# Lornatang/Real_ESRGAN-PyTorch

Measured on AMD Instinct MI355X. Metric: x4 SR train images/sec (256->1024), higher is better.
Workload: dtype f16; 1 GPU; RealESRNet x4 L1 train step, RRDBNet 23 blocks, LR 256^2 -> HR 1024^2, batch 16/GPU, degradation=hip, Adam+EMA, GradScaler; global_batch=16, parallelism=dp1

## Files before the change

include/resr.h:

```cpp
#ifndef RESR_H_
#define RESR_H_

#include <stddef.h>
#include <stdint.h>

#ifdef __cplusplus
extern "C" {
#endif

#define RESR_VERSION 3

typedef enum {
    RESR_OK = 0,
    RESR_ERR_ARG = -1,
    RESR_ERR_LAUNCH = -2,
    RESR_ERR_WORKSPACE = -3
} resr_status;

typedef enum { RESR_F16 = 0, RESR_F32 = 1, RESR_F16X2 = 2 } resr_dtype;

enum {
    RESR_CONV_LRELU = 1 << 0,
    RESR_CONV_UPSAMPLE_IN = 1 << 1,
    RESR_CONV_CLAMP01 = 1 << 2,
    RESR_CONV_OUT_NCHW_F32 = 1 << 3,
    RESR_CONV_MASK = 1 << 4,
    RESR_CONV_NO_BIAS = 1 << 5,
    RESR_CONV_AUX_BEFORE_MASK = 1 << 6,
    RESR_CONV_AUX_BEFORE_RES = 1 << 7,
    RESR_CONV_WRITE_SIGNBITS = 1 << 8,
    RESR_CONV_MASK_BITS = 1 << 9,
    RESR_CONV_OUT_SINGLE = 1 << 10,
    RESR_CONV_SINGLE_W16 = 1 << 11,
    RESR_CONV_MX_PAIRS = 1 << 12,
    RESR_CONV_MX_SIGNBITS = 1 << 13
};

typedef struct {
    int32_t n, h, w;
    int32_t cin;
    int32_t cin0;
    int32_t in0_stride;
    int32_t in1_stride;
    int32_t cout;
    int32_t cout_pad;
    int32_t out_stride;
    int32_t res0_stride, res1_stride, mask_stride;
    int32_t dtype;
    int32_t flags;
    float s0, t0, s1, t1, slope;
    int32_t in0_chunk_stride, in1_chunk_stride, out_chunk_stride;
    int32_t res0_chunk_stride, res1_chunk_stride, mask_chunk_stride;
    int64_t in0_lo_offset, in1_lo_offset, out_lo_offset, res0_lo_offset, res1_lo_offset;
    int32_t s2d_in_channels, s2d_out_channels, cout_groups;
    int32_t x2_pair_chunks;
    int32_t reserved2_;
    int64_t mask_lo_offset;
    int64_t in0_q_offset, in1_q_offset, out_q_offset, w_mx_offset;
// ... 370 lines not shown
```

real_esrgan-pytorch_amd/csrc/common.h:

```cpp
#pragma once
#include <hip/hip_runtime.h>
#include <stdint.h>
#include <stdio.h>
#include <stdlib.h>
#include <string.h>

#include <type_traits>

#include "resr.h"
#include "resr_debug.h"

namespace resr {

typedef _Float16 half_t;
typedef _Float16 half4 __attribute__((ext_vector_type(4)));
typedef _Float16 half8 __attribute__((ext_vector_type(8)));
typedef float float4v __attribute__((ext_vector_type(4)));
typedef unsigned uint2v __attribute__((ext_vector_type(2)));
typedef float float16v __attribute__((ext_vector_type(16)));

char* err_buf();
int fail(int code, const char* fmt, ...);

#define RESR_CHECK_LAUNCH(name)                                                        \
    do {                                                                               \
        hipError_t e_ = hipGetLastError();                                             \
        if (e_ != hipSuccess) return fail(RESR_ERR_LAUNCH, "%s: %s", name, hipGetErrorString(e_)); \
    } while (0)

bool prof_on();
void prof_before(hipStream_t st);
void prof_after(hipStream_t st, int kernel_id, double flop, double bytes = 0.0);

inline size_t elem_size(int dtype) { return dtype == RESR_F32 ? 4 : 2; }
inline size_t act_tensors(int dtype) { return dtype == RESR_F16X2 ? 2 : 1; }
constexpr float kLoScale = 4096.f, kLoInv = 1.f / 4096.f;
constexpr int kMaxDevices = 16;
inline size_t align_up(size_t v, size_t a) { return (v + a - 1) / a * a; }
inline bool no_pad_skip() { return getenv("RESR_NO_PAD_SKIP") != nullptr; }
inline bool degrade_parent_kernels() { return getenv("RESR_DEGRADE_PARENT_KERNELS") != nullptr; }

template <typename F>
inline bool with_scale(int s, F&& f) {
    switch (s) {
        case 1: f(std::integral_constant<int, 1>()); return true;
        case 2: f(std::integral_constant<int, 2>()); return true;
        case 3: f(std::integral_constant<int, 3>()); return true;
        case 4: f(std::integral_constant<int, 4>()); return true;
        default: return false;
    }
}

__device__ __forceinline__ void split_f16(float v, half_t& hi, half_t& lo) {
    hi = (half_t)v;
    lo = (half_t)((v - (float)hi) * kLoScale);
}

constexpr int kPrescaleBackoffStep = 4, kPrescaleBackoffMax = 40;
__host__ __device__ __forceinline__ bool grad_prescale_lifted(unsigned amax_bits) {
    const unsigned e = (amax_bits >> 23) & 0xffu;
    return e != 0u && e < 127u;
}
__host__ __device__ __forceinline__ float grad_prescale(unsigned amax_bits, bool inverse) {
// ... 58 lines not shown
```

real_esrgan-pytorch_amd/csrc/conv3x3.h:

```cpp
#pragma once
#include "host_api.h"

namespace resr {

struct ConvArgs {
    const char* in0;
    const char* in1;
    const char* w;
    const float* bias;
    const char* res0;
    const char* res1;
    const char* mask;
    char* out;
    uint8_t* aux;
    int n, h, w_, hs, ws;
    int cin, cin0;
    int in0_stride_b, in1_stride_b;
    int cout;
    int out_stride, res0_stride, res1_stride, mask_stride;
    size_t in0_chunk_b, in1_chunk_b;
    int out_chunk, res0_chunk, res1_chunk, mask_chunk;
    int flags;
    float s0, t0, s1, t1, slope;
    int tiles_x, tiles_y;
// ... 34 lines not shown
constexpr int kMaxChain = 6;
constexpr int kMaxBiasGroups = 8;
constexpr int kChainHdr = 16;
struct ChainArgs {
    int njobs;
    unsigned cap;
    unsigned* state;
    unsigned* host_errors;
    const char* nan16;
    int split[kMaxChain + 2];
    ChainJob job[kMaxChain];
};
struct ChainNone {};

bool conv3x3_ws_supported(const ConvArgs& a);
int conv3x3_ws_f16(const ConvArgs& a, int mt, bool x2, hipStream_t stream);
int conv3x3_ws_chain_f16(const ConvArgs& a, const ChainJob* jobs, int njobs, const double* flop, const double* bytes, bool x2, void* state, size_t state_bytes, hipStream_t stream);
int conv3x3_ws_mt1(const ConvArgs& a, int tile_rows, hipStream_t stream);
int conv3x3_ws_mt2(const ConvArgs& a, int tile_rows, hipStream_t stream);
int conv3x3_ws_x2_mt1(const ConvArgs& a, int tile_rows, hipStream_t stream);
int conv3x3_ws_x2_mt2(const ConvArgs& a, int tile_rows, hipStream_t stream);
int conv3x3_ws_mx_mt1(const ConvArgs& a, int tile_rows, hipStream_t stream);
int conv3x3_ws_mx_mt2(const ConvArgs& a, int tile_rows, hipStream_t stream);
int conv3x3_ws_sparse(const ConvArgs& a, int tile_rows, int sp, bool x2, hipStream_t stream);
int conv3x3_ws_chain_launch(const ConvArgs& a, const ChainArgs& cj, int tile_rows, int kind, bool x2, double flop, double bytes, hipStream_t stream);
int conv3x3_ws_chain_launch_x2(const ConvArgs& a, const ChainArgs& cj, int tile_rows, int kind, double flop, double bytes, hipStream_t stream);
int conv3x3_ws_chain_launch_mx(const ConvArgs& a, const ChainArgs& cj, int tile_rows, int kind, double flop, double bytes, hipStream_t stream);

inline ResrConvDesc conv_desc_base(int n, int h, int w, int dtype, int flags, float slope) {
    ResrConvDesc c;
    memset(&c, 0, sizeof(c));
    c.n = n; c.h = h; c.w = w; c.dtype = dtype; c.flags = flags;
    c.s0 = c.t0 = c.s1 = c.t1 = 1.f; c.slope = slope;
    return c;
}

inline double conv_algorithmic_bytes(const ConvArgs& a, size_t es) {
    const double px_out = (double)a.n * a.h * a.w_, px_in = (double)a.n * a.hs * a.ws;
    const int pair_ch = (es == 4 && a.pair_chunks > 0 && a.pair_chunks * 32 < a.cin) ? a.pair_chunks * 32 : a.cin;
    double b = px_in * (pair_ch * (double)es + (a.cin - pair_ch) * 2.0);
    const bool nchw = a.flags & RESR_CONV_OUT_NCHW_F32;
    b += px_out * a.cout * (nchw ? 4 : (es == 4 && a.out_single) ? 2 : es);
    if (a.flags & RESR_CONV_MASK) b += px_out * ((a.flags & RESR_CONV_MASK_BITS) ? ((a.cout + 31) / 32) * 4.0 : a.cout * (double)es);
    if (a.res0) b += px_out * a.cout * es;
    if (a.res1) b += px_out * a.cout * es;
    if (a.out_q) b += px_out * a.cout * 2.0;
    if (a.aux) b += px_out * ((a.flags & RESR_CONV_WRITE_SIGNBITS) ? ((a.cout + 31) / 32) * 4.0 : nchw ? a.cout : a.cout * (double)es);
    return b;
}

template <int SPP>
__device__ __forceinline__ int swz(int hx) {
    if constexpr (SPP == 4) return (hx >> 2) & 3;
    else return (hx >> 1) & 7;
}

template <typename T>
struct Frag;
template <>
struct Frag<half_t> {
    static __device__ __forceinline__ float16v mma(const uint4& a, const uint4& b, float16v c) {
        return __builtin_amdgcn_mfma_f32_32x32x16_f16(__builtin_bit_cast(half8, a),
                                                      __builtin_bit_cast(half8, b), c, 0, 0, 0);
    }
    static __device__ __forceinline__ float ld(const char* p, int idx) {
        return (float)reinterpret_cast<const half_t*>(p)[idx];
// ... 44 lines not shown
```

real_esrgan-pytorch_amd/csrc/conv3x3.hip:

```cpp
#include <stdlib.h>

#include <type_traits>

#include "conv3x3.h"
#include "packed_layout.h"

namespace resr {

template <typename T, int MT, int NT, int NW>
__global__ __launch_bounds__(64 * NW) void conv3x3_kernel(const ConvArgs a) {
    constexpr int NTHR = 64 * NW;
    constexpr int E = 16 / (int)sizeof(T);
    constexpr int SPP = 32 / E;
    constexpr int KS = SPP / 2;
    constexpr int PB = 32 * (int)sizeof(T);
    constexpr int TH = NW * NT, TW = 32, HH = TH + 2, HW = TW + 2;
    constexpr int NSLOT = HH * HW * SPP;
    constexpr int NS = (NSLOT + NTHR - 1) / NTHR;
    constexpr int BUF = HH * HW * PB;
    constexpr int WTAP = KS * MT * 1024;

    extern __shared__ __attribute__((aligned(16))) char smem[];

    const int tid = threadIdx.x, lane = tid & 63, wave = tid >> 6;
// ... 239 lines not shown
                        const float* bias, const void* res0, const void* res1, const void* mask,
                        void* out, void* aux, ConvArgs& a) {
    if (!d || !in0 || !w || !out) return fail(RESR_ERR_ARG, "conv3x3: null argument");
    if (d->cin <= 0 || (d->cin & 31) || (d->cin0 & 31) || d->cin0 <= 0 || d->cin0 > d->cin)
        return fail(RESR_ERR_ARG, "conv3x3: cin=%d cin0=%d must be positive multiples of 32", d->cin, d->cin0);
    if (d->cin0 < d->cin && !in1) return fail(RESR_ERR_ARG, "conv3x3: in1 missing for cin0 < cin");
    if (d->cout_pad != 32 && d->cout_pad != 64) return fail(RESR_ERR_ARG, "conv3x3: cout_pad=%d", d->cout_pad);
    if (d->cout <= 0 || d->cout > d->cout_pad) return fail(RESR_ERR_ARG, "conv3x3: cout=%d", d->cout);
    if (!(d->flags & RESR_CONV_OUT_NCHW_F32) && (d->cout & 3))
        return fail(RESR_ERR_ARG, "conv3x3: NHWC output needs cout %% 4 == 0");
    if (d->n <= 0 || d->h <= 0 || d->w <= 0) return fail(RESR_ERR_ARG, "conv3x3: empty shape");
    if ((d->flags & RESR_CONV_UPSAMPLE_IN) && ((d->h | d->w) & 1))
        return fail(RESR_ERR_ARG, "conv3x3: upsampled input needs even h,w");
    if ((d->flags & RESR_CONV_MASK) && !mask) return fail(RESR_ERR_ARG, "conv3x3: mask missing");
    if (d->flags & RESR_CONV_WRITE_SIGNBITS) {
        if (!aux || (d->cout & 7) || res0 || res1 ||
            (d->flags & (RESR_CONV_MASK | RESR_CONV_OUT_NCHW_F32 | RESR_CONV_CLAMP01 | RESR_CONV_AUX_BEFORE_MASK | RESR_CONV_AUX_BEFORE_RES)))
            return fail(RESR_ERR_ARG, "conv3x3: WRITE_SIGNBITS needs aux_out, cout %% 8 == 0 and a plain (bias/LeakyReLU) epilogue");
    }
    if (d->flags & RESR_CONV_MASK_BITS) {
        if (!(d->flags & RESR_CONV_MASK) || (d->cout & 7) || res0 || res1 || aux ||
            (d->flags & (RESR_CONV_OUT_NCHW_F32 | RESR_CONV_CLAMP01 | RESR_CONV_WRITE_SIGNBITS)))
            return fail(RESR_ERR_ARG, "conv3x3: MASK_BITS goes with MASK, cout %% 8 == 0, no residuals / aux");
    }
    const size_t es = elem_size(d->dtype);
    memset(&a, 0, sizeof(a));
    a.in0 = (const char*)in0; a.in1 = (const char*)in1; a.w = (const char*)w; a.bias = bias;
    a.res0 = (const char*)res0; a.res1 = (const char*)res1; a.mask = (const char*)mask;
    a.out = (char*)out; a.aux = (uint8_t*)aux;
    a.n = d->n; a.h = d->h; a.w_ = d->w;
    const bool up = d->flags & RESR_CONV_UPSAMPLE_IN;
    a.hs = up ? d->h / 2 : d->h; a.ws = up ? d->w / 2 : d->w;
    a.cin = d->cin; a.cin0 = d->cin0;
    a.in0_stride_b = (int)(d->in0_stride * es); a.in1_stride_b = (int)(d->in1_stride * es);
    a.cout = d->cout; a.out_stride = d->out_stride;
    a.res0_stride = d->res0_stride; a.res1_stride = d->res1_stride; a.mask_stride = d->mask_stride;
    auto chunk = [](int32_t v) { return v > 0 ? v : 32; };
    a.in0_chunk_b = (size_t)chunk(d->in0_chunk_stride) * es; a.in1_chunk_b = (size_t)chunk(d->in1_chunk_stride) * es;
    a.out_chunk = chunk(d->out_chunk_stride); a.res0_chunk = chunk(d->res0_chunk_stride);
    a.res1_chunk = chunk(d->res1_chunk_stride); a.mask_chunk = chunk(d->mask_chunk_stride);
    a.flags = d->flags & ~(RESR_CONV_OUT_SINGLE | RESR_CONV_SINGLE_W16 | RESR_CONV_MX_PAIRS | RESR_CONV_MX_SIGNBITS); a.s0 = d->s0; a.t0 = d->t0; a.s1 = d->s1; a.t1 = d->t1; a.slope = d->slope;
    a.s2d_c = 0; a.tap_c = 0; a.ngroups = 1; a.w_group_b = 0;
    a.pair_chunks = d->cin / 32; a.out_single = 0;
    a.mask_lo = (d->dtype == RESR_F16X2 && mask && (d->flags & RESR_CONV_MASK) && !(d->flags & RESR_CONV_MASK_BITS)) ? (long)d->mask_lo_offset : 0L;
    if (a.mask_lo < 0) return fail(RESR_ERR_ARG, "conv3x3: mask_lo_offset=%ld", a.mask_lo);
    if (d->dtype == RESR_F16X2) {
// ... 76 lines not shown
    const void* res0 = a.res0;
    const void* res1 = a.res1;
    const int groups = d->cout_groups > 1 ? d->cout_groups : 1;
    (void)have_bias;
    const int mt = d->cout_pad / 32;
    if (d->dtype == RESR_F16X2) {
        const bool nchw = d->flags & RESR_CONV_OUT_NCHW_F32;
        const bool in1_pairs = in1 && d->cin0 < d->cin && a.pair_chunks * 32 > d->cin0;
        if (d->in0_lo_offset == 0 || (in1_pairs && d->in1_lo_offset == 0) || (!nchw && !a.out_single && d->out_lo_offset == 0) ||
            (res0 && d->res0_lo_offset == 0) || (res1 && d->res1_lo_offset == 0))
            return fail(RESR_ERR_ARG, "conv3x3: RESR_F16X2 needs the hi -> lo offset of every pair operand");
        a.in0_lo_b = (size_t)d->in0_lo_offset * es; a.in1_lo_b = (size_t)d->in1_lo_offset * es;
        a.out_lo = a.out_single ? 0L : (long)d->out_lo_offset; a.res0_lo = (long)d->res0_lo_offset; a.res1_lo = (long)d->res1_lo_offset;
        if (!conv3x3_ws_supported(a))
            return fail(RESR_ERR_ARG, "conv3x3: RESR_F16X2 needs tensors below 4 GB / 2^24 pixels and cout %% 8 == 0");
        if (a.mx && (a.s2d_c > 0 || a.tap_c > 0)) return fail(RESR_ERR_ARG, "conv3x3: RESR_CONV_MX_PAIRS with sparse taps");
        return conv3x3_ws_f16(a, mt, true, stream);
    }
    const long tiles4 = (long)((d->w + 31) / 32) * ((d->h + 15) / 16) * d->n;
    const bool big = tiles4 >= 512;
    if (d->dtype == RESR_F16) {
        static const char* old_env = getenv("RESR_CONV_ONE_ROLE");
        if (!old_env && conv3x3_ws_supported(a)) return conv3x3_ws_f16(a, mt, false, stream);
        if (groups > 1) return fail(RESR_ERR_ARG, "conv3x3: cout_groups > 1 needs the producer/consumer kernel's preconditions");
        if (mt == 1) return big ? launch_conv<half_t, 1, 2, 8>(a, stream) : launch_conv<half_t, 1, 2, 4>(a, stream);
        return launch_conv<half_t, 2, 2, 4>(a, stream);
    } else if (d->dtype == RESR_F32) {
        if (mt == 1) return launch_conv<float, 1, 2>(a, stream);
        return launch_conv<float, 2, 2>(a, stream);
    }
    return fail(RESR_ERR_ARG, "conv3x3: dtype=%d", d->dtype);
}

int conv3x3_block_dispatch(int njobs, const ResrConvDesc* d, const void* in0, const void* in1, const void* const* w,
                           const float* const* bias, const void* const* mask, void* const* out, void* const* aux,
                           const ResrConvDesc* d5, const void* w5, const float* bias5, const void* res0_5, const void* res1_5,
                           void* out5, void* chain_state, size_t chain_state_bytes, hipStream_t stream) {
    if (njobs <= 0 || njobs > 4 || !d) return fail(RESR_ERR_ARG, "conv3x3_chain: njobs=%d", njobs);
    ConvArgs a[4], a5;
    for (int j = 0; j < njobs; ++j) {
        const int rc = conv3x3_args(&d[j], in0, in1, w[j], bias ? bias[j] : nullptr, nullptr, nullptr, mask ? mask[j] : nullptr,
                                    out[j], aux ? aux[j] : nullptr, a[j]);
        if (rc) return rc;
    }
    if (d5) {
        const int rc = conv3x3_args(d5, in0, in1, w5, bias5, res0_5, res1_5, nullptr, out5, nullptr, a5);
// ... 129 lines not shown
```

real_esrgan-pytorch_amd/csrc/conv3x3_ws.h:

```cpp
#pragma once
#include <stdlib.h>

#include <type_traits>

#include "conv3x3.h"

#ifndef RESR_TIMING_TAPS
#define RESR_TIMING_TAPS 9
#endif
#if defined(RESR_TRACE) && RESR_TRACE == 2
#define RESR_TRACE_STAMPS 192
#else
#define RESR_TRACE_STAMPS 64
#endif
#ifndef RESR_TIMING_VALU
#define RESR_TIMING_VALU 0
#endif

namespace resr {

static __device__ uint4 g_conv_zero16 = {0, 0, 0, 0};

extern unsigned long long* g_conv_trace;

// ... 176 lines not shown
    if (wave == 0 || wave == NWC) stamp(wave == 0 ? 1 : 0);

    float* bias_lds = reinterpret_cast<float*>(smem + C::NHB * BUF);
    if (wave == 0) {
        const bool f_bias = !(a.flags & RESR_CONV_NO_BIAS) && a.bias != nullptr;
        bias_lds[lane] = (f_bias && lane < a.cout) ? a.bias[lane] * (X2 ? kLoScale : 1.f) : 0.f;
    }
    if constexpr (MT == 2 && CH == 0) {
        if (a.ngroups > 1 && !(a.flags & RESR_CONV_NO_BIAS) && a.bias != nullptr) {
            float* gb = reinterpret_cast<float*>(smem + C::GB_OFF);
            for (int i = tid; i < a.ngroups * 64 && i < kMaxBiasGroups * 64; i += C::NTHR)
                gb[i] = a.bias[i] * (X2 ? kLoScale : 1.f);
        }
    }
    if constexpr (CH) {
        float* cb = reinterpret_cast<float*>(smem + C::CHAIN_OFF);
        if (wave < kMaxChain && lane < 32) {
            const float* bp = wave < cj.njobs ? cj.job[wave].bias : nullptr;
            cb[wave * 32 + lane] = (bp && !(a.flags & RESR_CONV_NO_BIAS) && lane < a.cout) ? bp[lane] * (X2 ? kLoScale : 1.f) : 0.f;
        }
        if (wave == 0 && lane == 0) *reinterpret_cast<unsigned*>(smem + C::CHAIN_OFF + kMaxChain * 128) = 0u;
    }
    constexpr bool FAST = EPI == 0 || EPI == 2 || EPI == 6 || EPI == 16 || EPI == 33 || EPI == 128;
    if constexpr (EPI == 128) {
        if (wave == 1) reinterpret_cast<float*>(smem + C::LUT_OFF)[lane] = lane < a.cout ? a.prelu[lane] : 0.f;
    }
    if constexpr (FAST && EPI == 33) {
        if (wave == 1 && lane < 16) {
            float4v m;
#pragma unroll
            for (int r = 0; r < 4; ++r) m[r] = (((lane >> r) & 1) ? 1.f : a.slope) * (X2 ? kLoInv : 1.f);
            *reinterpret_cast<float4v*>(smem + C::LUT_OFF + lane * 16) = m;
        }
    }
    if (wave >= NWC) {
        const int pw = wave - NWC;
        if constexpr (C::NHB == 3) {
            const int ups3 = (a.flags & RESR_CONV_UPSAMPLE_IN) ? 1 : 0;
            constexpr int REM = NI - (NIP - 1) * NP;
            static_assert(NIP < 64, "vmcnt is 6 bits");
            unsigned cst[NIP], pix[NIP];
            unsigned long long val[NIP], inb[NIP];
            const unsigned lds_base = (unsigned)(size_t)(__attribute__((address_space(3))) char*)smem;
            auto dma_s = [&](const char* sbase, unsigned voff, unsigned dst, unsigned long long mask) {
                unsigned long long save;
                asm volatile("s_mov_b64 %0, exec\n\ts_mov_b64 exec, %1\n\ts_mov_b32 m0, %2\n\ts_nop 0\n\t"
// ... 433 lines not shown
    int pend_tile = 0;
    unsigned pend_tag = 0;
    const int njobs_c = [&] { if constexpr (CH) return cj.njobs; else return 1; }();
    auto publish = [&]() {
        if constexpr (CH) {
            if (pend) {
                asm volatile("s_waitcnt vmcnt(0)" ::: "memory");
                if (lane == 0) {
                    unsigned* cnt = reinterpret_cast<unsigned*>(smem + C::CHAIN_OFF + kMaxChain * 128);
                    const unsigned old = __hip_atomic_fetch_add(cnt, 1u, __ATOMIC_RELAXED, __HIP_MEMORY_SCOPE_WORKGROUP);
                    if ((old % NWC) == NWC - 1)
                        __hip_atomic_store(cj.state + kChainHdr + pend_tile, pend_tag, __ATOMIC_RELAXED, __HIP_MEMORY_SCOPE_AGENT);
                }
                pend = false;
            }
        }
    };
    int c_tx = 0, c_ty = 0, c_n = 0, c_grp = 0;
    const int s_tx = tile_step % a.tiles_x, s_t2 = tile_step / a.tiles_x;
    const int s_ty = s_t2 % a.tiles_y, s_n = s_t2 / a.tiles_y;
    for (int job = (CH == 3 ? pin_job : 0); job < (CH == 3 ? pin_job + 1 : njobs_c); ++job) {
    if constexpr (CH) nchunks = stages_of(cj.job[job].cin);
    for (int tile = first; tile < tile_end; tile += tile_step) {
        if constexpr (FAST) {
            if (tile == first) {
                const int t2 = first / a.tiles_x;
                c_tx = first % a.tiles_x;
                c_ty = t2 % a.tiles_y;
                c_n = t2 / a.tiles_y;
            } else {
                c_tx += s_tx;
                if (c_tx >= a.tiles_x) { c_tx -= a.tiles_x; ++c_ty; }
                c_ty += s_ty;
                if (c_ty >= a.tiles_y) { c_ty -= a.tiles_y; ++c_n; }
                c_n += s_n;
            }
            c_grp = 0;
            if (MT == 2 && a.ngroups > 1) c_grp = c_n / a.n;
        }
        unsigned mword[EPI == 33 ? NT : 1][MT];
        bool own_top = true;
        if constexpr (CH == 2) own_top = cj.job[job].kind != 3;
        if constexpr (EPI == 33) if (own_top) {
            int x, y0, n;
            if constexpr (FAST) {
                x = c_tx * TW + (lane & 31);
                y0 = c_ty * TH + row0;
                n = c_n - c_grp * a.n;
            } else {
                const int tsp = tile % ntiles_sp;
                x = (tsp % a.tiles_x) * TW + (lane & 31);
                y0 = ((tsp / a.tiles_x) % a.tiles_y) * TH + row0;
                n = tsp / (a.tiles_x * a.tiles_y);
            }
            const unsigned xc = (unsigned)(x < a.w_ ? x : a.w_ - 1);
            const unsigned wpp = (unsigned)((a.cout + 31) >> 5);
#pragma unroll
            for (int t = 0; t < NT; ++t) {
                const int y = y0 + t;
                const unsigned p = ((unsigned)n * a.h + (unsigned)(y < a.h ? y : a.h - 1)) * a.w_ + xc;
#pragma unroll
                for (int m = 0; m < MT; ++m) {
                    const unsigned* mk = reinterpret_cast<const unsigned*>(a.mask);
                    if constexpr (CH) mk = reinterpret_cast<const unsigned*>(cj.job[job].aux);
                    mword[t][m] = mk[(size_t)p * wpp + (m < (int)wpp ? m : 0)];
                }
            }
        }
        auto run_stage = [&](int ck, auto is_mx_c) {
            constexpr bool IS_MX = decltype(is_mx_c)::value;
            if (wave == 0) stamp(1);
            asm volatile("s_barrier" ::: "memory");
            if (wave == 0) stamp(1);
            const char* lbuf = smem + hbc * BUF;
            const int wsel = (!CH && nchunks <= C::NWB && ntiles == ntiles_sp) ? ck : par;
            constexpr int PP = (NWC == 4 || MT * NT * 16 + (NT + 2) * 8 <= 112) ? 1 : 0;
            uint4 rowf[PP + 1][NT + 2];
            auto rload = [&](int slot, int gi) {
                const char* bp = lbuf + boff[gi % 3][gi / 3];
#pragma unroll
                for (int r = 0; r < NT + 2; ++r) rowf[slot][r] = *reinterpret_cast<const uint4*>(bp + r * (HW * PB));
            };
            if constexpr (IS_MX) {
                {
                    static_assert(KS == 2, "MX stage: 64-byte pixel records");
                    typedef int v8i __attribute__((ext_vector_type(8)));
                    typedef int v4i __attribute__((ext_vector_type(4)));
                    const char* wl = wlds + wsel * C::WBUF;
                    const int one = 0x7f7f7f7f;
                    auto ld8 = [&](const char* p0, const char* p1) -> v8i {
// ... 111 lines not shown
                                    asm volatile("v_pk_add_f16 %0, %0, %1" : "+v"(timing_valu[v & 3]) : "v"(timing_valu[(v + 1) & 3]));
                            }
                    }
                    __builtin_amdgcn_sched_barrier(0);
                }
            }
            par ^= 1;
            if (!st_keeps_halo(ck)) hbc = hbc + 1 == C::NHB ? 0 : hbc + 1;
            if (wave == 0) stamp(1);
            if constexpr (CH) publish();
        };
        {
            int ck = 0;
            if constexpr (MX) {
                const int npair = nchunks < x2_p3 ? nchunks : x2_p3;
                for (; ck < npair; ck += 2) {
                    run_stage(ck, std::false_type{});
                    run_stage(ck + 1, std::true_type{});
                }
            }
            for (; ck < nchunks; ++ck) run_stage(ck, std::false_type{});
        }

        if constexpr (FAST) {
            const size_t goff = MT == 2 ? (size_t)c_grp * 64 : 0;
            const int x0 = c_tx * TW;
            const int y0 = c_ty * TH;
            const int n = c_n - c_grp * a.n;
            typedef const ConvArgs __attribute__((address_space(4))) * KernargPtr;
            KernargPtr ep = (KernargPtr)__builtin_amdgcn_kernarg_segment_ptr();
            asm volatile("" : "+s"(ep));
            struct {
                const char *res0, *res1;
                char* out;
                uint8_t* aux;
                int h, w_, cout, out_stride, res0_stride, res1_stride, flags;
                int out_chunk, res0_chunk, res1_chunk;
                float s0, t0, s1, t1, slope;
                long out_lo, res0_lo, res1_lo;
                long out_q;
            } e;
            e.out_q = 0;
            if constexpr (X2) e.out_q = ep->out_q;
            if constexpr (CH && X2) e.out_q = cj.job[job].out_q;
            e.out = ep->out; e.h = ep->h; e.w_ = ep->w_; e.cout = ep->cout; e.out_stride = ep->out_stride;
            e.out_chunk = ep->out_chunk; e.flags = ep->flags; e.slope = ep->slope;
// ... 545 lines not shown
```

real_esrgan-pytorch_amd/csrc/conv3x3_ws.hip:

```cpp
#include <stdlib.h>

#include <mutex>

#include "conv3x3.h"

namespace resr {

unsigned long long* g_conv_trace = nullptr;
void conv_trace_set(void* p) { g_conv_trace = (unsigned long long*)p; }

bool conv3x3_chain_device_ok() {
    static int ok_dev[kMaxDevices] = {0};
    int dev = 0;
    if (hipGetDevice(&dev) != hipSuccess || dev < 0 || dev >= kMaxDevices) return false;
    if (!ok_dev[dev]) {
        hipDeviceProp_t prop;
        ok_dev[dev] = (hipGetDeviceProperties(&prop, dev) == hipSuccess && prop.multiProcessorCount == 256) ? 1 : -1;
    }
    return ok_dev[dev] > 0;
}

bool conv3x3_ws_supported(const ConvArgs& a) {
    const size_t px = (size_t)a.n * a.hs * a.ws;
    const size_t stride = (size_t)(a.in0_stride_b > a.in1_stride_b ? a.in0_stride_b : a.in1_stride_b);
// ... 94 lines not shown
            if (c.owned && c.owner != stream && hipStreamWaitEvent(stream, c.ev, 0) != hipSuccess)
                return fail(RESR_ERR_LAUNCH, "conv3x3_chain: hipStreamWaitEvent");
            c.owner = stream;
            c.owned = true;
        }
        cj.state = (unsigned*)state;
        cj.cap = (unsigned)(state_bytes / sizeof(unsigned) - kChainHdr);
        cj.host_errors = c.err_dev;
        cj.nan16 = c.nan16;
        cj.njobs = njobs;
        memcpy(cj.split, split, sizeof(split));
        double f = 0, b = 0;
        for (int j = 0; j < njobs; ++j) { cj.job[j] = jobs[j]; f += flop[j]; b += bytes[j]; }
        for (int j = njobs; j < kMaxChain; ++j) cj.job[j] = jobs[njobs - 1];
        const int kind = (a.flags & RESR_CONV_MASK_BITS) ? 2 : (a.flags & RESR_CONV_WRITE_SIGNBITS) ? 1 : 0;
        const int rc = conv3x3_ws_chain_launch(a, cj, rows, kind, x2, f, b, stream);
        if (rc == RESR_OK && !capturing && hipEventRecord(c.ev, stream) != hipSuccess) return fail(RESR_ERR_LAUNCH, "conv3x3_chain: hipEventRecord");
        return rc;
    }
}

int conv3x3_ws_f16(const ConvArgs& a, int mt, bool x2, hipStream_t stream) {
    static const int rows1[] = {16, 8}, rows2[] = {16, 8};
    if (mt == 2 && (a.s2d_c > 0 || a.tap_c > 0) && !a.res0 && !a.res1 && !a.mask && !a.aux &&
        !(a.flags & ~(RESR_CONV_LRELU | RESR_CONV_NO_BIAS)) && a.cin0 == a.cin && (!(a.flags & RESR_CONV_LRELU) || (a.slope >= 0.f && a.slope <= 1.f)))
        return conv3x3_ws_sparse(a, 8, a.s2d_c > 0 ? 1 : 2, x2, stream);
    if (x2 && a.mx) {
        if (mt == 1) return conv3x3_ws_mx_mt1(a, pick_rows(a, rows1, 2), stream);
        return conv3x3_ws_mx_mt2(a, pick_rows(a, rows2, 2), stream);
    }
    if (x2) {
        if (mt == 1) return conv3x3_ws_x2_mt1(a, pick_rows(a, rows1, 2), stream);
        return conv3x3_ws_x2_mt2(a, pick_rows(a, rows2, 2), stream);
    }
    if (mt == 1) return conv3x3_ws_mt1(a, pick_rows(a, rows1, 2), stream);
    return conv3x3_ws_mt2(a, pick_rows(a, rows2, 2), stream);
}

}
```

real_esrgan-pytorch_amd/csrc/generator.hip:

```cpp
#include <stdlib.h>
#include <vector>

#include "conv3x3.h"
#include "packed_layout.h"

namespace resr {

namespace {

struct ConvSpec {
    int cout, cin, cin_pad, cout_pad;
    size_t w_off, b_off;
    size_t pk_fwd, pk_bwd;
};

struct X2Plan {
    bool mx_train;
    bool mx;
    bool growth_single, growth_w16;
    bool f16_backward;
    bool mx_bwd;
    bool mx_wgrad;
    bool mx_tail;
    bool gg_single;
// ... 572 lines not shown
    auto MXT = [&](ResrConvDesc& cd, size_t pk_off, long in_q, long out_q) {
        if (!xp.mx_tail) return;
        cd.flags |= RESR_CONV_MX_PAIRS;
        cd.in0_q_offset = in_q; cd.out_q_offset = out_q;
        cd.w_mx_offset = (int64_t)((pk_mx + pk_off * 2) - (pk + pk_off * wes));
    };
    {
        const ConvSpec& c = p.convs[p.i_conv4];
        RUN(wgrad(c, H4, W4, b.c3, 64, 32, b.g4, 32, 0, 1.f, pl4, 0, lo_4, lo_g4, xp.mx_tail ? 2 * lo_4 : 0, xp.mx_tail ? 2 * lo_g4 : 0));
        ResrConvDesc cd = dgrad(H4, W4, 32, 32, 32, 0, 64, 64, 32, RESR_CONV_MASK | RESR_CONV_MASK_BITS, lo_g4, 0, lo_4);
        cd.out_chunk_stride = pl4;
        MXT(cd, c.pk_bwd, 2 * lo_g4, 2 * lo_4);
        RUN(conv3x3_dispatch(&cd, b.g4, nullptr, pk + c.pk_bwd * wes, nullptr, nullptr, nullptr, b.bits_c3, b.gA, nullptr, st));
    }
    {
        const ConvSpec& c = p.convs[p.i_conv3];
        RUN(wgrad(c, H4, W4, b.u2, 64, 32, b.gA, 32, 0, 1.f, pl4, pl4, lo_4, lo_4, xp.mx_tail ? 2 * lo_4 : 0, xp.mx_tail ? 2 * lo_4 : 0));
        ResrConvDesc cd = dgrad(H4, W4, 64, 32, 64, 0, 64, 64, 32, RESR_CONV_MASK | RESR_CONV_MASK_BITS, lo_4, 0, lo_4);
        cd.in0_chunk_stride = pl4; cd.out_chunk_stride = pl4;
        MXT(cd, c.pk_bwd, 2 * lo_4, 2 * lo_4);
        RUN(conv3x3_dispatch(&cd, b.gA, nullptr, pk + c.pk_bwd * wes, nullptr, nullptr, nullptr, b.bits_u2, b.gB, nullptr, st));
    }
    if (debug_stop() == 1) return RESR_OK;
    {
        const ConvSpec& c = p.convs[p.i_up2];
        RUN(wgrad(c, H4, W4, b.u1, 64, 32, b.gB, 32, RESR_CONV_UPSAMPLE_IN, 1.f, pl2, pl4, lo_2, lo_4, xp.mx_tail ? 2 * lo_2 : 0, xp.mx_tail ? 2 * lo_4 : 0));
        ResrConvDesc cd = dgrad(H4, W4, 64, 32, 64, 0, 64, 64, 32, 0, lo_4, 0, lo_4);
        cd.in0_chunk_stride = pl4; cd.out_chunk_stride = pl4;
        MXT(cd, c.pk_bwd, 2 * lo_4, 0);
        RUN(conv3x3_dispatch(&cd, b.gB, nullptr, pk + c.pk_bwd * wes, nullptr, nullptr, nullptr, nullptr, b.gA, nullptr, st));
        for (int q = 0; q < 2; ++q)
            RUN(sumpool2x2_dispatch(b.gA + (size_t)q * pl4 * es, b.gM1 + (size_t)q * pl2 * es, b.u1 + (size_t)q * pl2 * es,
                                    N, H2, W2, 32, dt, 0.2f, st, lo_4, lo_2));
    }
    if (debug_stop() == 2) return RESR_OK;
    {
        const ConvSpec& c = p.convs[p.i_up1];
        RUN(wgrad(c, H2, W2, b.feat, 64, 32, b.gM1, 32, RESR_CONV_UPSAMPLE_IN, 1.f, plane, pl2, lo_t, lo_2));
        ResrConvDesc cd = dgrad(H2, W2, 64, 32, 64, 0, 64, 64, 32, 0, lo_2, 0, lo_2);
        cd.in0_chunk_stride = pl2; cd.out_chunk_stride = pl2;
        RUN(conv3x3_dispatch(&cd, b.gM1, nullptr, pk + c.pk_bwd * wes, nullptr, nullptr, nullptr, nullptr, b.gA, nullptr, st));
        for (int q = 0; q < 2; ++q)
            RUN(sumpool2x2_dispatch(b.gA + (size_t)q * pl2 * es, b.gF + (size_t)q * plane * es, nullptr, N, h, w, 32, dt, 0.2f, st,
                                    lo_2, lo_t));
    }
    if (debug_stop() == 3) return RESR_OK;
    int cur = 0;
    {
        const ConvSpec& c = p.convs[p.i_conv2];
        RUN(wgrad(c, h, w, b.trunk_out, 64, 32, b.gF, 32, 0, 1.f, plane, plane, lo_t, lo_t));
        ResrConvDesc cd = dgrad(h, w, 64, 32, 64, 0, 64, 64, 32, 0, lo_t, 0, lo_t);
        cd.in0_chunk_stride = plane; cd.out_chunk_stride = plane;
        if (xp.mx_bwd) cd.out_q_offset = 2 * lo_t;
        RUN(conv3x3_dispatch(&cd, b.gF, nullptr, pk + c.pk_bwd * wes, nullptr, nullptr, nullptr, nullptr, b.gT[0], nullptr, st));
    }
    auto MXB = [&](ResrConvDesc& cd, size_t pk_off, long out_q) {
        if (!xp.mx_bwd) return;
        cd.flags |= RESR_CONV_MX_PAIRS;
        cd.x2_pair_chunks = 0;
        cd.in0_q_offset = 2 * lo_t; cd.in1_q_offset = 2 * lo_gs; cd.out_q_offset = out_q;
        cd.w_mx_offset = (int64_t)((pk_mx + pk_off * 2) - (pk + pk_off * wes));
    };
    RUN(ready(0));
    int e_idx = 0;
    const bool batch_rrdb = 78 * wm <= kWgradMaxJobs && !getenv("RESR_WGRAD_PER_BLOCK");
    WgradConv wc[15];
    for (int r = p.nrdb - 1; r >= 0; --r) {
// ... 72 lines not shown
```

Measured before the change: 135.5 images/sec.

## Fuse 2x2 sum-pool into upsample dgrad epilogue and add planar output epilogue

The backward data-gradient convs of the two nearest-upsample layers now pool 2x2 neighbours directly in the conv epilogue. They combine lanes via DPP and row pairs in registers, then apply the saved-activation leaky-ReLU mask before storing the quarter-size gradient. This avoids writing the full-resolution gradient to memory and running separate sumpool kernels. A planar NCHW f32 epilogue is also added for small-cout output convs. Both paths add constrained new kernel variants and change the fp16 rounding order of the pooled sums.

```diff
diff --git a/include/resr.h b/include/resr.h
--- a/include/resr.h
+++ b/include/resr.h
@@ -33,7 +33,8 @@
     RESR_CONV_OUT_SINGLE = 1 << 10,
     RESR_CONV_SINGLE_W16 = 1 << 11,
     RESR_CONV_MX_PAIRS = 1 << 12,
-    RESR_CONV_MX_SIGNBITS = 1 << 13
+    RESR_CONV_MX_SIGNBITS = 1 << 13,
+    RESR_CONV_POOL2_OUT = 1 << 14
 };
 
 typedef struct {
diff --git a/real_esrgan-pytorch_amd/csrc/common.h b/real_esrgan-pytorch_amd/csrc/common.h
--- a/real_esrgan-pytorch_amd/csrc/common.h
+++ b/real_esrgan-pytorch_amd/csrc/common.h
@@ -39,6 +39,7 @@
 inline size_t align_up(size_t v, size_t a) { return (v + a - 1) / a * a; }
 inline bool no_pad_skip() { return getenv("RESR_NO_PAD_SKIP") != nullptr; }
 inline bool degrade_parent_kernels() { return getenv("RESR_DEGRADE_PARENT_KERNELS") != nullptr; }
+inline bool no_tail_epilogues() { return getenv("RESR_NO_TAIL_EPILOGUES") != nullptr; }
 
 template <typename F>
 inline bool with_scale(int s, F&& f) {
diff --git a/real_esrgan-pytorch_amd/csrc/conv3x3.h b/real_esrgan-pytorch_amd/csrc/conv3x3.h
--- a/real_esrgan-pytorch_amd/csrc/conv3x3.h
+++ b/real_esrgan-pytorch_amd/csrc/conv3x3.h
@@ -80,6 +80,8 @@
 int conv3x3_ws_x2_mt2(const ConvArgs& a, int tile_rows, hipStream_t stream);
 int conv3x3_ws_mx_mt1(const ConvArgs& a, int tile_rows, hipStream_t stream);
 int conv3x3_ws_mx_mt2(const ConvArgs& a, int tile_rows, hipStream_t stream);
+int conv3x3_ws_pool2(const ConvArgs& a, hipStream_t stream);
+int conv3x3_ws_planar(const ConvArgs& a, int tile_rows, hipStream_t stream);
 int conv3x3_ws_sparse(const ConvArgs& a, int tile_rows, int sp, bool x2, hipStream_t stream);
 int conv3x3_ws_chain_launch(const ConvArgs& a, const ChainArgs& cj, int tile_rows, int kind, bool x2, double flop, double bytes, hipStream_t stream);
 int conv3x3_ws_chain_launch_x2(const ConvArgs& a, const ChainArgs& cj, int tile_rows, int kind, double flop, double bytes, hipStream_t stream);
@@ -98,8 +100,9 @@
     const int pair_ch = (es == 4 && a.pair_chunks > 0 && a.pair_chunks * 32 < a.cin) ? a.pair_chunks * 32 : a.cin;
     double b = px_in * (pair_ch * (double)es + (a.cin - pair_ch) * 2.0);
     const bool nchw = a.flags & RESR_CONV_OUT_NCHW_F32;
-    b += px_out * a.cout * (nchw ? 4 : (es == 4 && a.out_single) ? 2 : es);
-    if (a.flags & RESR_CONV_MASK) b += px_out * ((a.flags & RESR_CONV_MASK_BITS) ? ((a.cout + 31) / 32) * 4.0 : a.cout * (double)es);
+    const double px_st = (a.flags & RESR_CONV_POOL2_OUT) ? px_out * 0.25 : px_out;
+    b += px_st * a.cout * (nchw ? 4 : (es == 4 && a.out_single) ? 2 : es);
+    if (a.flags & RESR_CONV_MASK) b += px_st * ((a.flags & RESR_CONV_MASK_BITS) ? ((a.cout + 31) / 32) * 4.0 : a.cout * (double)es);
     if (a.res0) b += px_out * a.cout * es;
     if (a.res1) b += px_out * a.cout * es;
     if (a.out_q) b += px_out * a.cout * 2.0;
diff --git a/real_esrgan-pytorch_amd/csrc/conv3x3.hip b/real_esrgan-pytorch_amd/csrc/conv3x3.hip
--- a/real_esrgan-pytorch_amd/csrc/conv3x3.hip
+++ b/real_esrgan-pytorch_amd/csrc/conv3x3.hip
@@ -285,6 +285,13 @@
         if (!(d->flags & RESR_CONV_MASK) || (d->cout & 7) || res0 || res1 || aux ||
             (d->flags & (RESR_CONV_OUT_NCHW_F32 | RESR_CONV_CLAMP01 | RESR_CONV_WRITE_SIGNBITS)))
             return fail(RESR_ERR_ARG, "conv3x3: MASK_BITS goes with MASK, cout %% 8 == 0, no residuals / aux");
+    }
+    if (d->flags & RESR_CONV_POOL2_OUT) {
+        if (d->dtype != RESR_F16 || d->cout != 64 || d->cout_pad != 64 || ((d->h | d->w) & 1) || res0 || res1 || aux ||
+            d->cout_groups > 1 || d->s2d_in_channels > 0 || d->s2d_out_channels > 0 ||
+            (d->flags & (RESR_CONV_LRELU | RESR_CONV_CLAMP01 | RESR_CONV_OUT_NCHW_F32 | RESR_CONV_AUX_BEFORE_MASK | RESR_CONV_AUX_BEFORE_RES |
+                         RESR_CONV_WRITE_SIGNBITS | RESR_CONV_MASK_BITS | RESR_CONV_MX_PAIRS)))
+            return fail(RESR_ERR_ARG, "conv3x3: POOL2_OUT is an f16 pass of cout = cout_pad = 64 with even h, w and a plain (bias / saved-activation mask) epilogue");
     }
     const size_t es = elem_size(d->dtype);
     memset(&a, 0, sizeof(a));
@@ -407,6 +414,7 @@
     if (d->dtype == RESR_F16) {
         static const char* old_env = getenv("RESR_CONV_ONE_ROLE");
         if (!old_env && conv3x3_ws_supported(a)) return conv3x3_ws_f16(a, mt, false, stream);
+        if (d->flags & RESR_CONV_POOL2_OUT) return fail(RESR_ERR_ARG, "conv3x3: POOL2_OUT needs the producer/consumer kernel's preconditions");
         if (groups > 1) return fail(RESR_ERR_ARG, "conv3x3: cout_groups > 1 needs the producer/consumer kernel's preconditions");
         if (mt == 1) return big ? launch_conv<half_t, 1, 2, 8>(a, stream) : launch_conv<half_t, 1, 2, 4>(a, stream);
         return launch_conv<half_t, 2, 2, 4>(a, stream);
diff --git a/real_esrgan-pytorch_amd/csrc/conv3x3_ws.h b/real_esrgan-pytorch_amd/csrc/conv3x3_ws.h
--- a/real_esrgan-pytorch_amd/csrc/conv3x3_ws.h
+++ b/real_esrgan-pytorch_amd/csrc/conv3x3_ws.h
@@ -222,6 +222,10 @@
         if (wave == 0 && lane == 0) *reinterpret_cast<unsigned*>(smem + C::CHAIN_OFF + kMaxChain * 128) = 0u;
     }
     constexpr bool FAST = EPI == 0 || EPI == 2 || EPI == 6 || EPI == 16 || EPI == 33 || EPI == 128;
+    constexpr bool POOL = EPI == 256 || EPI == 257, PLANAR = EPI == 512;
+    static_assert(!POOL || (MT == 2 && NT == 4 && NWC == 4 && X2 == 0 && SP == 0 && CH == 0 && sizeof(T) == 2), "pooled store: the 16-row cout-64 f16 shape");
+    static_assert(!PLANAR || (MT == 1 && X2 == 0 && SP == 0 && CH == 0), "planar epilogue: cout <= 32 shapes, plain f16");
+    constexpr bool WALK = FAST || POOL || PLANAR;
     if constexpr (EPI == 128) {
         if (wave == 1) reinterpret_cast<float*>(smem + C::LUT_OFF)[lane] = lane < a.cout ? a.prelu[lane] : 0.f;
     }
@@ -701,7 +705,7 @@
     for (int job = (CH == 3 ? pin_job : 0); job < (CH == 3 ? pin_job + 1 : njobs_c); ++job) {
     if constexpr (CH) nchunks = stages_of(cj.job[job].cin);
     for (int tile = first; tile < tile_end; tile += tile_step) {
-        if constexpr (FAST) {
+        if constexpr (WALK) {
             if (tile == first) {
                 const int t2 = first / a.tiles_x;
                 c_tx = first % a.tiles_x;
@@ -745,6 +749,25 @@
                     mword[t][m] = mk[(size_t)p * wpp + (m < (int)wpp ? m : 0)];
                 }
             }
+        }
+        constexpr int PMK_TOP = 2;
+        uint4v pmk[EPI == 257 ? 2 : 1][EPI == 257 ? MT : 1][2];
+        auto pmk_request = [&](int tp) {
+            if constexpr (EPI == 257) {
+                const int x = c_tx * TW + (lane & 31);
+                const int y = c_ty * TH + row0 + 2 * tp;
+                const unsigned cellp = ((unsigned)c_n * ((unsigned)a.h >> 1) + ((unsigned)(y < a.h ? y : a.h - 1) >> 1)) * ((unsigned)a.w_ >> 1) +
+                                       ((unsigned)(x < a.w_ ? x : a.w_ - 1) >> 1);
+#pragma unroll
+                for (int m = 0; m < MT; ++m)
+#pragma unroll
+                    for (int j = 0; j < 2; ++j)
+                        pmk[tp][m][j] = *reinterpret_cast<const uint4v*>(a.mask + ((size_t)cellp * a.mask_stride + (size_t)m * a.mask_chunk + j * 16) * 2 + (lane >> 5) * 16);
+            }
+        };
+        if constexpr (EPI == 257) {
+#pragma unroll
+            for (int tp = 0; tp < PMK_TOP; ++tp) pmk_request(tp);
         }
         auto run_stage = [&](int ck, auto is_mx_c) {
             constexpr bool IS_MX = decltype(is_mx_c)::value;
@@ -902,6 +925,136 @@
             for (; ck < nchunks; ++ck) run_stage(ck, std::false_type{});
         }
 
+        if constexpr (POOL) {
+            const int x0 = c_tx * TW, y0 = c_ty * TH, n = c_n;
+            typedef const ConvArgs __attribute__((address_space(4))) * KernargPtr;
+            KernargPtr ep = (KernargPtr)__builtin_amdgcn_kernarg_segment_ptr();
+            asm volatile("" : "+s"(ep));
+            struct {
+                char* out;
+                int h, w_, out_stride, out_chunk;
+                float slope;
+            } e;
+            e.out = ep->out; e.h = ep->h; e.w_ = ep->w_; e.out_stride = ep->out_stride; e.out_chunk = ep->out_chunk;
+            if constexpr (EPI == 257) e.slope = ep->slope;
+            int lane_e = lane;
+            asm volatile("" : "+v"(lane_e));
+            const int lx_e = lane_e & 31, kh_e = lane_e >> 5;
+            const int x = x0 + lx_e;
+            const unsigned hp = (unsigned)e.h >> 1, wp = (unsigned)e.w_ >> 1;
+            const unsigned xp = (unsigned)(x < e.w_ ? x : e.w_ - 1) >> 1;
+            const unsigned kh16 = (unsigned)kh_e * 16u;
+            auto cell = [&](int tp) {
+                const int y = y0 + row0 + 2 * tp;
+                return ((unsigned)n * hp + ((unsigned)(y < e.h ? y : e.h - 1) >> 1)) * wp + xp;
+            };
+            asm volatile("s_nop 7\n\ts_nop 7\n\ts_nop 3");
+            if constexpr (EPI == 257) {
+#pragma unroll
+                for (int tp = PMK_TOP; tp < 2; ++tp) pmk_request(tp);
+#pragma unroll
+                for (int tp = 0; tp < 2; ++tp)
+#pragma unroll
+                    for (int m = 0; m < MT; ++m)
+#pragma unroll
+                        for (int j = 0; j < 2; ++j) asm volatile("" : "+v"(pmk[tp][m][j]));
+            }
+#pragma unroll
+            for (int tp = 0; tp < 2; ++tp) {
+                const int y = y0 + row0 + 2 * tp;
+                const bool st = y < e.h && x < e.w_ && !(lx_e & 1);
+                char* const orow = e.out + (size_t)cell(tp) * e.out_stride * 2 + kh16;
+#pragma unroll
+                for (int m = 0; m < MT; ++m)
+#pragma unroll
+                    for (int j = 0; j < 2; ++j) {
+                        unsigned own[2][4], nb[2][4];
+#pragma unroll
+                        for (int r = 0; r < 2; ++r) {
+                            float16v& A = acc[m][2 * tp + r];
+                            float v0 = A[8 * j + 0], v1 = A[8 * j + 1], v2 = A[8 * j + 2], v3 = A[8 * j + 3];
+                            float v4 = A[8 * j + 4], v5 = A[8 * j + 5], v6 = A[8 * j + 6], v7 = A[8 * j + 7];
+                            permlane32_swap4(v0, v1, v2, v3, v4, v5, v6, v7);
+                            const float2v q[4] = {{v0, v1}, {v2, v3}, {v4, v5}, {v6, v7}};
+#pragma unroll
+                            for (int k = 0; k < 4; ++k) {
+                                own[r][k] = __builtin_bit_cast(unsigned, __builtin_convertvector(q[k], half2v));
+                                nb[r][k] = (unsigned)__builtin_amdgcn_update_dpp(0, (int)own[r][k], 0xB1, 0xF, 0xF, true);
+                            }
+                        }
+                        uint4v d;
+#pragma unroll
+                        for (int k = 0; k < 4; ++k) {
+                            const unsigned o0 = own[0][k], n0 = nb[0][k], o1 = own[1][k], n1 = nb[1][k];
+                            const float2v a00 = __builtin_convertvector(__builtin_bit_cast(half2v, o0), float2v);
+                            const float2v a01 = __builtin_convertvector(__builtin_bit_cast(half2v, n0), float2v);
+                            const float2v a10 = __builtin_convertvector(__builtin_bit_cast(half2v, o1), float2v);
+                            const float2v a11 = __builtin_convertvector(__builtin_bit_cast(half2v, n1), float2v);
+                            float2v s;
+#pragma unroll
+                            for (int c = 0; c < 2; ++c) {
+                                float u = 0.f;
+                                u += a00[c];
+                                u += a01[c];
+                                u += a10[c];
+                                u += a11[c];
+                                s[c] = u;
+                            }
+                            if constexpr (EPI == 257) {
+                                const unsigned mw = pmk[tp][m][j][k];
+                                const float2v mf = __builtin_convertvector(__builtin_bit_cast(half2v, mw), float2v);
+                                s[0] *= mf[0] > 0.f ? 1.f : e.slope;
+                                s[1] *= mf[1] > 0.f ? 1.f : e.slope;
+                            }
+                            d[k] = __builtin_bit_cast(unsigned, __builtin_convertvector(s, half2v));
+                        }
+                        if (st) *reinterpret_cast<uint4v*>(orow + ((size_t)m * e.out_chunk + j * 16) * 2) = d;
+                    }
+            }
+            group_bias(tile + tile_step);
+            init_acc();
+            if (wave == 0) stamp(1);
+            continue;
+        }
+        if constexpr (PLANAR) {
+            const int x0 = c_tx * TW, y0 = c_ty * TH, n = c_n;
+            typedef const ConvArgs __attribute__((address_space(4))) * KernargPtr;
+            KernargPtr ep = (KernargPtr)__builtin_amdgcn_kernarg_segment_ptr();
+            asm volatile("" : "+s"(ep));
+            struct {
+                char* out;
+                uint8_t* aux;
+                int h, w_, cout, flags;
+            } e;
+            e.out = ep->out; e.aux = ep->aux; e.h = ep->h; e.w_ = ep->w_; e.cout = ep->cout; e.flags = ep->flags;
+            int lane_e = lane;
+            asm volatile("" : "+v"(lane_e));
+            const int x = x0 + (lane_e & 31);
+            const bool f_clamp = e.flags & RESR_CONV_CLAMP01;
+            asm volatile("s_nop 7\n\ts_nop 7\n\ts_nop 3");
+            float* const o = reinterpret_cast<float*>(e.out);
+#pragma unroll
+            for (int t = 0; t < NT; ++t) {
+                const int y = y0 + row0 + t;
+                if (lane_e < 32 && y < e.h && x < e.w_) {
+#pragma unroll
+                    for (int c = 0; c < 4; ++c) {
+                        if (c >= e.cout) continue;
+                        const size_t q = (((size_t)n * e.cout + c) * e.h + y) * e.w_ + x;
+                        float u = acc[0][t][c];
+                        if (f_clamp) {
+                            if (e.aux) e.aux[q] = (u >= 0.f && u <= 1.f) ? 1 : 0;
+                            u = u < 0.f ? 0.f : (u > 1.f ? 1.f : u);
+                        }
+                        o[q] = u;
+                    }
+                }
+            }
+            group_bias(tile + tile_step);
+            init_acc();
+            if (wave == 0) stamp(1);
+            continue;
+        }
         if constexpr (FAST) {
             const size_t goff = MT == 2 ? (size_t)c_grp * 64 : 0;
             const int x0 = c_tx * TW;
diff --git a/real_esrgan-pytorch_amd/csrc/conv3x3_ws.hip b/real_esrgan-pytorch_amd/csrc/conv3x3_ws.hip
--- a/real_esrgan-pytorch_amd/csrc/conv3x3_ws.hip
+++ b/real_esrgan-pytorch_amd/csrc/conv3x3_ws.hip
@@ -140,6 +140,15 @@
 
 int conv3x3_ws_f16(const ConvArgs& a, int mt, bool x2, hipStream_t stream) {
     static const int rows1[] = {16, 8}, rows2[] = {16, 8};
+    if (a.flags & RESR_CONV_POOL2_OUT) {
+        if (x2 || mt != 2 || a.s2d_c > 0 || a.tap_c > 0 || a.ngroups > 1 || a.res0 || a.res1 || a.aux || a.prelu || ((a.h | a.w_) & 1) ||
+            ((a.flags & RESR_CONV_MASK) && !a.mask))
+            return fail(RESR_ERR_ARG, "conv3x3: POOL2_OUT is a plain f16 pass of one 64-channel output group");
+        return conv3x3_ws_pool2(a, stream);
+    }
+    if (!x2 && mt == 1 && (a.flags & RESR_CONV_OUT_NCHW_F32) && a.cout <= 4 && !a.res0 && !a.res1 && !a.mask && !a.prelu && a.ngroups == 1 &&
+        !(a.flags & ~(RESR_CONV_OUT_NCHW_F32 | RESR_CONV_CLAMP01 | RESR_CONV_NO_BIAS | RESR_CONV_UPSAMPLE_IN)) && !no_tail_epilogues())
+        return conv3x3_ws_planar(a, pick_rows(a, rows1, 2), stream);
     if (mt == 2 && (a.s2d_c > 0 || a.tap_c > 0) && !a.res0 && !a.res1 && !a.mask && !a.aux &&
         !(a.flags & ~(RESR_CONV_LRELU | RESR_CONV_NO_BIAS)) && a.cin0 == a.cin && (!(a.flags & RESR_CONV_LRELU) || (a.slope >= 0.f && a.slope <= 1.f)))
         return conv3x3_ws_sparse(a, 8, a.s2d_c > 0 ? 1 : 2, x2, stream);
diff --git a/real_esrgan-pytorch_amd/csrc/conv3x3_ws_tail.hip b/real_esrgan-pytorch_amd/csrc/conv3x3_ws_tail.hip
--- /dev/null
+++ b/real_esrgan-pytorch_amd/csrc/conv3x3_ws_tail.hip
@@ -0,0 +1,15 @@
+#include "conv3x3_ws.h"
+
+namespace resr {
+
+int conv3x3_ws_pool2(const ConvArgs& a, hipStream_t stream) {
+    if ((a.flags & RESR_CONV_MASK) && a.mask) return launch_ws_epi<half_t, 2, 4, 4, 257>(a, stream);
+    return launch_ws_epi<half_t, 2, 4, 4, 256>(a, stream);
+}
+
+int conv3x3_ws_planar(const ConvArgs& a, int tile_rows, hipStream_t stream) {
+    if (tile_rows >= 16) return launch_ws_epi<half_t, 1, 2, 8, 512>(a, stream);
+    return launch_ws_epi<half_t, 1, 1, 8, 512>(a, stream);
+}
+
+}
diff --git a/real_esrgan-pytorch_amd/csrc/generator.hip b/real_esrgan-pytorch_amd/csrc/generator.hip
--- a/real_esrgan-pytorch_amd/csrc/generator.hip
+++ b/real_esrgan-pytorch_amd/csrc/generator.hip
@@ -618,16 +618,24 @@
         RUN(conv3x3_dispatch(&cd, b.gA, nullptr, pk + c.pk_bwd * wes, nullptr, nullptr, nullptr, b.bits_u2, b.gB, nullptr, st));
     }
     if (debug_stop() == 1) return RESR_OK;
+    const size_t px4 = (size_t)N * H4 * W4;
+    const bool pool_out = dt == RESR_F16 && !no_tail_epilogues() && px4 <= (1u << 24) && px4 * 64 + 64 < (1ull << 32) && !getenv("RESR_CONV_ONE_ROLE");
     {
         const ConvSpec& c = p.convs[p.i_up2];
         RUN(wgrad(c, H4, W4, b.u1, 64, 32, b.gB, 32, RESR_CONV_UPSAMPLE_IN, 1.f, pl2, pl4, lo_2, lo_4, xp.mx_tail ? 2 * lo_2 : 0, xp.mx_tail ? 2 * lo_4 : 0));
         ResrConvDesc cd = dgrad(H4, W4, 64, 32, 64, 0, 64, 64, 32, 0, lo_4, 0, lo_4);
         cd.in0_chunk_stride = pl4; cd.out_chunk_stride = pl4;
         MXT(cd, c.pk_bwd, 2 * lo_4, 0);
-        RUN(conv3x3_dispatch(&cd, b.gB, nullptr, pk + c.pk_bwd * wes, nullptr, nullptr, nullptr, nullptr, b.gA, nullptr, st));
-        for (int q = 0; q < 2; ++q)
-            RUN(sumpool2x2_dispatch(b.gA + (size_t)q * pl4 * es, b.gM1 + (size_t)q * pl2 * es, b.u1 + (size_t)q * pl2 * es,
-                                    N, H2, W2, 32, dt, 0.2f, st, lo_4, lo_2));
+        if (pool_out && debug_stop() != 2) {
+            cd.flags |= RESR_CONV_POOL2_OUT | RESR_CONV_MASK;
+            cd.out_chunk_stride = pl2; cd.mask_stride = 32; cd.mask_chunk_stride = pl2; cd.slope = 0.2f;
+            RUN(conv3x3_dispatch(&cd, b.gB, nullptr, pk + c.pk_bwd * wes, nullptr, nullptr, nullptr, b.u1, b.gM1, nullptr, st));
+        } else {
+            RUN(conv3x3_dispatch(&cd, b.gB, nullptr, pk + c.pk_bwd * wes, nullptr, nullptr, nullptr, nullptr, b.gA, nullptr, st));
+            for (int q = 0; q < 2; ++q)
+                RUN(sumpool2x2_dispatch(b.gA + (size_t)q * pl4 * es, b.gM1 + (size_t)q * pl2 * es, b.u1 + (size_t)q * pl2 * es,
+                                        N, H2, W2, 32, dt, 0.2f, st, lo_4, lo_2));
+        }
     }
     if (debug_stop() == 2) return RESR_OK;
     {
@@ -635,10 +643,16 @@
         RUN(wgrad(c, H2, W2, b.feat, 64, 32, b.gM1, 32, RESR_CONV_UPSAMPLE_IN, 1.f, plane, pl2, lo_t, lo_2));
         ResrConvDesc cd = dgrad(H2, W2, 64, 32, 64, 0, 64, 64, 32, 0, lo_2, 0, lo_2);
         cd.in0_chunk_stride = pl2; cd.out_chunk_stride = pl2;
-        RUN(conv3x3_dispatch(&cd, b.gM1, nullptr, pk + c.pk_bwd * wes, nullptr, nullptr, nullptr, nullptr, b.gA, nullptr, st));
-        for (int q = 0; q < 2; ++q)
-            RUN(sumpool2x2_dispatch(b.gA + (size_t)q * pl2 * es, b.gF + (size_t)q * plane * es, nullptr, N, h, w, 32, dt, 0.2f, st,
-                                    lo_2, lo_t));
+        if (pool_out && debug_stop() != 3) {
+            cd.flags |= RESR_CONV_POOL2_OUT;
+            cd.out_chunk_stride = plane;
+            RUN(conv3x3_dispatch(&cd, b.gM1, nullptr, pk + c.pk_bwd * wes, nullptr, nullptr, nullptr, nullptr, b.gF, nullptr, st));
+        } else {
+            RUN(conv3x3_dispatch(&cd, b.gM1, nullptr, pk + c.pk_bwd * wes, nullptr, nullptr, nullptr, nullptr, b.gA, nullptr, st));
+            for (int q = 0; q < 2; ++q)
+                RUN(sumpool2x2_dispatch(b.gA + (size_t)q * pl2 * es, b.gF + (size_t)q * plane * es, nullptr, N, h, w, 32, dt, 0.2f, st,
+                                        lo_2, lo_t));
+        }
     }
     if (debug_stop() == 3) return RESR_OK;
     int cur = 0;
```

After: 136.4 images/sec (median of 6 runs). About the same (+0.6%).
